# awkrail/svpc

Measured on AMD Instinct MI355X. Metric: train steps/sec (vivt, batch=16, clip_seq=12), higher is better.
Workload: dtype bf16x3; 1 GPU; MODEL_TYPE=vivt train step: N=16 videos/GPU x S=12 clips x Lv=100 frames x F=3072, Lt=22, D=768, H=12, L=6 (enc+step-enc+dec), V=951, A=384, E=10; dropout .1/.1/.4; fwd+bwd+allreduce+clip+BertAdam; mode=bf16x3, global_batch=16, parallelism=dp1, launch=hipGraph replay, gpus_requested=1

## Files before the change

include/svpc_hip.h:

```cpp
#ifndef SVPC_HIP_H
#define SVPC_HIP_H
#include <stddef.h>
#ifdef __cplusplus
extern "C" {
#endif

typedef struct ihipStream_t* svpc_stream_t;
typedef unsigned long long svpc_u64;

#define SVPC_ACT_NONE 0
#define SVPC_ACT_RELU 1
#define SVPC_ACT_GELU 2
#define SVPC_ACT_SIGMOID 3

const char* svpc_last_error(void);
int svpc_abi_version(void);

int svpc_ln_fwd(const float* x, const int* src_rows, const float* res, const float* gamma, const float* beta, float* y,
                float* mean, float* rstd, int R, int D, float eps, float p_pre, unsigned site_pre, float p_post,
                unsigned site_post, const svpc_u64* seed, const float* add1, int mod1, const float* add2, const int* idx2,
                svpc_stream_t stream);
int svpc_ln_fwd_t(const void* x, int x_dt, const int* src_rows, const void* res, const float* gamma, const float* beta, void* y,
                  int y_dt, float* mean, float* rstd, int R, int D, float eps, float p_pre, unsigned site_pre, float p_post,
                  unsigned site_post, const svpc_u64* seed, const float* add1, int mod1, const float* add2, const int* idx2,
// ... 46 lines not shown
                   int K, const float* bias, int act, float p_drop, unsigned site, const svpc_u64* seed, int accumulate,
                   float* workspace, size_t workspace_bytes, svpc_stream_t stream);
int svpc_gemm_glds_r(const void* A, int lda, int a_kc, const void* B, int ldb, int b_kc, void* C, int c_dt, int ldc, void* Z, const void* R,
                     int M, int N, int K, const float* bias, int act, float p_drop, unsigned site, const svpc_u64* seed, int accumulate,
                     float* workspace, size_t workspace_bytes, svpc_stream_t stream);
int svpc_gemm_glds_rg(const void* A, int lda, int a_kc, const void* B, int ldb, int b_kc, void* C, int c_dt, int ldc, void* Z, const void* R,
                      const void* G, int gact, int M, int N, int K, const float* bias, int act, float p_drop, unsigned site,
                      const svpc_u64* seed, int accumulate, float* workspace, size_t workspace_bytes, svpc_stream_t stream);
int svpc_gemm_p8(const void* A, int lda, const void* B, int ldb, void* C, int ldc, void* Z, int M, int N, int K, const float* bias, int act,
                 svpc_stream_t stream);
int svpc_gemm_p8x3_supported(int lda, int a_lo, int ldb, int ldc, int c_lo, int ldz, int M, int N, int K);
int svpc_gemm_p8x3(const void* A, int lda, int a_lo, const void* B, int ldb, long long b_lo, void* C, int ldc, int c_lo, void* Z, int ldz,
                   int M, int N, int K, const float* bias, int act, svpc_stream_t stream);
int svpc_gemm_s4x3(const void* A, int lda, int a_lo, const void* B, int ldb, long long b_lo, void* C, int ldc, int c_lo, void* Z, int ldz,
                   int M, int N, int K, const float* bias, int act, svpc_stream_t stream);
int svpc_gemm_s4t_supported(int lda, int ldb, int ldc, int M, int N, int K);
int svpc_gemm_s4t(const void* A, int lda, const void* B, int ldb, void* C, int ldc, const void* R, int M, int N, int K, svpc_stream_t stream);
int svpc_gemm_p8t_supported(int lda, int ldb, int ldc, int M, int N, int K);
int svpc_gemm_p8t(const void* A, int lda, const void* B, int ldb, void* C, int ldc, const void* G, int gact, const void* R, int M, int N, int K,
                  svpc_stream_t stream);
int svpc_gemm_l32_supported(int a_kc, int b_kc, int lda, int ldb, int M, int N, int K);
int svpc_gemm_l32_preferred(int a_kc, int b_kc, int lda, int ldb, int M, int N, int K);
int svpc_gemm_l32(const float* A, int lda, int a_kc, const float* B, int ldb, int b_kc, float* C, int ldc, float* Z, int M, int N, int K,
                  const float* bias, int act, float p_drop, unsigned site, const svpc_u64* seed, int accumulate, float* workspace,
                  size_t workspace_bytes, svpc_stream_t stream);
int svpc_gemm_l32_r(const float* A, int lda, int a_kc, const float* B, int ldb, int b_kc, float* C, int ldc, float* Z, const float* R, int M,
                    int N, int K, const float* bias, int act, float p_drop, unsigned site, const svpc_u64* seed, int accumulate,
                    float* workspace, size_t workspace_bytes, svpc_stream_t stream);
int svpc_gemm_l32_rg(const float* A, int lda, int a_kc, const float* B, int ldb, int b_kc, float* C, int ldc, const float* R, const float* G,
                     int gact, int M, int N, int K, int accumulate, float* workspace, size_t workspace_bytes, svpc_stream_t stream);
int svpc_gemm_l32_x3(const float* A, int lda, int a_kc, const float* B, int ldb, int b_kc, float* C, int ldc, float* Z, const float* R, int M,
                     int N, int K, const float* bias, int act, float p_drop, unsigned site, const svpc_u64* seed, int accumulate,
// ... 300 lines not shown
```

svpc_amd/csrc/gemm_s4t.hip:

```cpp
#include "gemm_common.h"
#include <stdlib.h>

typedef __bf16 bf16x8 __attribute__((ext_vector_type(8)));
typedef float floatx4 __attribute__((ext_vector_type(4)));
typedef short short4s __attribute__((ext_vector_type(4)));
typedef const void __attribute__((address_space(1))) * s4t_gptr;
typedef void __attribute__((address_space(3))) * s4t_lptr;

constexpr int S4T_BK = 64;
constexpr int S4T_HALF = 128 * S4T_BK * 2;
constexpr int S4T_STAGE = 2 * S4T_HALF;

__device__ __forceinline__ bf16x8 s4t_frag_tr(const char* __restrict__ a) {
    typedef short4s __attribute__((address_space(3))) * lds_ptr;
    const short4s lo = __builtin_amdgcn_ds_read_tr16_b64_v4i16((lds_ptr)(a));
    const short4s hi = __builtin_amdgcn_ds_read_tr16_b64_v4i16((lds_ptr)(a + 4 * 256));
    union { short s[8]; bf16x8 v; } u;
    u.s[0] = lo[0]; u.s[1] = lo[1]; u.s[2] = lo[2]; u.s[3] = lo[3];
    u.s[4] = hi[0]; u.s[5] = hi[1]; u.s[6] = hi[2]; u.s[7] = hi[3];
    return u.v;
}

template <bool HASR, int NS>
__global__ __launch_bounds__(512, NS == 2 ? 2 : 1) void gemm_s4t_kernel(const __bf16* __restrict__ A, int lda, const __bf16* __restrict__ B, int ldb,
                                                                        __bf16* __restrict__ C, int ldc, const __bf16* __restrict__ R, int M,
                                                                        int N, int K, int tiles_m, int tiles_n, int remap) {
    __shared__ __attribute__((aligned(1024))) char smem[NS * S4T_STAGE];
    const int wg = remap ? xcd_remap(blockIdx.x, tiles_m * tiles_n) : (int)blockIdx.x;
    const int tm = wg / tiles_n, tn = wg - tm * tiles_n;
    const int m0 = tm * 128, n0 = tn * 128;
    const int nk = K / S4T_BK;
    const int lane = threadIdx.x & 63, wave = __builtin_amdgcn_readfirstlane(threadIdx.x >> 6);
    const int wr = wave >> 1, wc = wave & 1;

    const int sr = lane >> 2, sc = (lane & 3) ^ (((lane >> 5) & 1) << 1);
    const __bf16* const ga = A + (size_t)min(m0 + 16 * wave + sr, M - 1) * lda + 8 * sc;
    const __bf16* gb[2];
#pragma unroll
    for (int u = 0; u < 2; ++u) {
        const int kr = 8 * wave + 4 * u + (lane >> 4);
        const int fx = 2 * ((kr & 3) | ((kr >> 1) & 4));
        const int col = min(n0 + 8 * ((lane & 15) ^ fx), N - 8);
        gb[u] = B + (size_t)kr * ldb + col;
    }
    const size_t stepB = (size_t)S4T_BK * ldb;
#define S4T_ISSUE(t)                                                                                                              \
    do {                                                                                                                          \
        char* st_ = smem + ((t) % NS) * S4T_STAGE;                                                                                \
        const __bf16* sa_ = ga + (size_t)(t) * S4T_BK;                                                                            \
        __builtin_amdgcn_global_load_lds((s4t_gptr)(sa_), (s4t_lptr)(st_ + ((wave * 2) << 10)), 16, 0, 0);                        \
        __builtin_amdgcn_global_load_lds((s4t_gptr)(sa_ + 32), (s4t_lptr)(st_ + ((wave * 2 + 1) << 10)), 16, 0, 0);               \
        __builtin_amdgcn_global_load_lds((s4t_gptr)(gb[0] + (size_t)(t) * stepB), (s4t_lptr)(st_ + S4T_HALF + wave * 2048), 16, 0, 0);        \
        __builtin_amdgcn_global_load_lds((s4t_gptr)(gb[1] + (size_t)(t) * stepB), (s4t_lptr)(st_ + S4T_HALF + wave * 2048 + 1024), 16, 0, 0); \
    } while (0)
    const int fr_off = (lane & 15) * 64 + ((((lane >> 4) ^ (((lane >> 3) & 1) << 1))) << 4);
#define S4T_FRAGA(img, blk, kb) (*reinterpret_cast<const bf16x8*>((img) + (((blk) * 2 + (kb)) << 10) + fr_off))
    const int tg = lane >> 4, tq = (lane & 15) >> 2, tp = lane & 3;
    const int tfx = 2 * (tq + 4 * (tg & 1));
    const int tb_off = (8 * tg + tq) * 256 + ((tp & 1) << 3);
    const int tp1 = tp >> 1;
#define S4T_FRAGB(img, cb, kb) s4t_frag_tr((img) + (kb) * (32 * 256) + tb_off + (((((2 * (cb)) ^ tfx)) | tp1) << 4))

    floatx4 acc[2][4];
#pragma unroll
    for (int i = 0; i < 2; ++i)
#pragma unroll
        for (int j = 0; j < 4; ++j) acc[i][j] = floatx4{0.f, 0.f, 0.f, 0.f};

#pragma unroll
    for (int t = 0; t < NS - 1; ++t)
        if (t < nk) S4T_ISSUE(t);
    for (int t = 0; t < nk; ++t) {
        if (NS == 4 && t + 2 < nk) asm volatile("s_waitcnt vmcnt(8)" ::: "memory");
        else if (NS >= 3 && t + 1 < nk) asm volatile("s_waitcnt vmcnt(4)" ::: "memory");
        else asm volatile("s_waitcnt vmcnt(0)" ::: "memory");
        __builtin_amdgcn_s_barrier();
        __builtin_amdgcn_sched_barrier(0);
        if (t + NS - 1 < nk) S4T_ISSUE(t + NS - 1);
        const char* sa = smem + (t % NS) * S4T_STAGE;
        const char* sb = sa + S4T_HALF;
#pragma unroll
        for (int kb = 0; kb < 2; ++kb) {
            bf16x8 bfr[4], afr[2];
#pragma unroll
            for (int j = 0; j < 4; ++j) bfr[j] = S4T_FRAGB(sb, wc * 4 + j, kb);
#pragma unroll
            for (int i = 0; i < 2; ++i) afr[i] = S4T_FRAGA(sa, wr * 2 + i, kb);
#pragma unroll
            for (int i = 0; i < 2; ++i)
#pragma unroll
                for (int j = 0; j < 4; ++j) acc[i][j] = __builtin_amdgcn_mfma_f32_16x16x32_bf16(bfr[j], afr[i], acc[i][j], 0, 0, 0);
        }
    }
#undef S4T_ISSUE
#undef S4T_FRAGA
#undef S4T_FRAGB
    __syncthreads();
    char* wl = smem + wave * 8192;
    const int row0 = m0 + wr * 32, col0 = n0 + wc * 64;
    const int l15 = lane & 15, q = lane >> 4;
    const int c8 = lane & 7, cc = col0 + 8 * c8, r0 = lane >> 3;
    const bool col_ok = cc + 8 <= N;
    bf16x8 rv[HASR ? 4 : 1];
#pragma unroll
    for (int it = 0; it < 4; ++it) {
        const int r = it * 8 + r0;
        if (HASR && col_ok && row0 + r < M) rv[it] = *reinterpret_cast<const bf16x8*>(R + (size_t)(row0 + r) * ldc + cc);
    }
#pragma unroll
    for (int i = 0; i < 2; ++i) {
        const int r = i * 16 + l15;
#pragma unroll
        for (int j = 0; j < 4; ++j) {
            const int c16 = j * 4 + q;
            *reinterpret_cast<floatx4*>(wl + r * 256 + ((c16 ^ (r & 7)) << 4)) = acc[i][j];
        }
    }
#pragma unroll
    for (int it = 0; it < 4; ++it) {
        const int r = it * 8 + r0;
        const floatx4 v0 = *reinterpret_cast<const floatx4*>(wl + r * 256 + (((2 * c8) ^ (r & 7)) << 4));
        const floatx4 v1 = *reinterpret_cast<const floatx4*>(wl + r * 256 + (((2 * c8 + 1) ^ (r & 7)) << 4));
        float v[8] = {v0[0], v0[1], v0[2], v0[3], v1[0], v1[1], v1[2], v1[3]};
        if (col_ok && row0 + r < M) {
            const size_t o = (size_t)(row0 + r) * ldc + cc;
            if (HASR) {
#pragma unroll
                for (int j = 0; j < 8; ++j) v[j] += (float)rv[it][j];
            }
            bf16x8 ov;
#pragma unroll
            for (int j = 0; j < 8; ++j) ov[j] = (__bf16)v[j];
            *reinterpret_cast<bf16x8*>(C + o) = ov;
        }
    }
}

extern "C" {

int svpc_gemm_s4t_supported(int lda, int ldb, int ldc, int M, int N, int K) {
    if (M <= 0 || N < 8 || K < S4T_BK || K % S4T_BK != 0 || (N & 7) != 0) return 0;
    if ((lda & 7) || (ldb & 7) || (ldc & 7) || lda < K || ldb < N || ldc < N) return 0;
    return 1;
}

int svpc_gemm_s4t(const void* A, int lda, const void* B, int ldb, void* C, int ldc, const void* R, int M, int N, int K, hipStream_t stream) {
    if (M <= 0 || N <= 0) return 0;
    SVPC_REQUIRE(svpc_gemm_s4t_supported(lda, ldb, ldc, M, N, K) == 1 &&
                     ((((uintptr_t)A) | ((uintptr_t)B) | ((uintptr_t)C) | ((uintptr_t)R)) & 15) == 0,
                 "gemm_s4t: needs K % 64 == 0, N % 8 == 0, 16-byte aligned bf16 rows");
    static int remap = -1, deep_max = -1;
    if (remap < 0) { const char* e = getenv("SVPC_GEMM_REMAP"); remap = e ? atoi(e) : 1; }
    if (deep_max < 0) { const char* e = getenv("SVPC_S4T_DEEP_MAX"); deep_max = e ? atoi(e) : 256; }
    const int tiles_m = ceil_div(M, 128), tiles_n = ceil_div(N, 128);
    const bool deep = tiles_m * tiles_n <= deep_max;
#define S4T_GO(RV, NSV)                                                                                                           \
    hipLaunchKernelGGL((gemm_s4t_kernel<RV, NSV>), dim3(tiles_m * tiles_n), dim3(512), 0, stream, (const __bf16*)A, lda, (const __bf16*)B, \
                       ldb, (__bf16*)C, ldc, (const __bf16*)R, M, N, K, tiles_m, tiles_n, remap)
    if (R != nullptr) { if (deep) S4T_GO(true, 4); else S4T_GO(true, 2); }
    else { if (deep) S4T_GO(false, 4); else S4T_GO(false, 2); }
#undef S4T_GO
    return svpc_check_launch("gemm_s4t");
}

}
```

svpc_amd/csrc/gemm_s4x3.hip:

```cpp
#include "gemm_common.h"
#include <stdlib.h>

typedef __bf16 bf16x8 __attribute__((ext_vector_type(8)));
typedef float floatx4 __attribute__((ext_vector_type(4)));
typedef const void __attribute__((address_space(1))) * s4_gptr;
typedef void __attribute__((address_space(3))) * s4_lptr;

constexpr int S4_BK = 64;
constexpr int S4_KS = 32;
constexpr int S4_HALF = 128 * S4_BK * 2;
constexpr int S4_STAGE = 2 * S4_HALF;

__device__ __forceinline__ uint32_t s4_pack2(float lo, float hi) {
    union { __bf16 h[2]; uint32_t u; } pk;
    pk.h[0] = (__bf16)lo; pk.h[1] = (__bf16)hi;
    return pk.u;
}
__device__ __forceinline__ float s4_lo(float v) { return v - (float)(__bf16)v; }
__device__ __forceinline__ float s4_gelu(float x) {
    const float u = x * 0.70710678118654752f, au = fabsf(u);
    const float t = __builtin_amdgcn_rcpf(fmaf(0.3275911f, au, 1.0f));
    float p = fmaf(1.061405429f, t, -1.453152027f);
    p = fmaf(p, t, 1.421413741f);
    p = fmaf(p, t, -0.284496736f);
    p = fmaf(p, t, 0.254829592f);
    const float e = __expf(-au * au);
    return 0.5f * x * (1.0f + copysignf(fmaf(-p * t, e, 1.0f), u));
}
template <int ACT>
__device__ __forceinline__ float s4_act(float z) {
    if (ACT == ACT_RELU) return fmaxf(z, 0.f);
    if (ACT == ACT_GELU) return s4_gelu(z);
    return z;
}

template <int ACT, int MODE>
__device__ __forceinline__ void s4_store_pass(const floatx4 (&acc)[2][4], __bf16* __restrict__ C, int ldc, const float4 (&bb)[4], int row0,
                                              int col0, int M, int N, int lane, char* __restrict__ wl) {
    const int l15 = lane & 15, q = lane >> 4;
#pragma unroll
    for (int i = 0; i < 2; ++i) {
        const int r = i * 16 + l15;
#pragma unroll
        for (int j = 0; j < 4; ++j) {
            float z0 = acc[i][j][0] + bb[j].x, z1 = acc[i][j][1] + bb[j].y, z2 = acc[i][j][2] + bb[j].z, z3 = acc[i][j][3] + bb[j].w;
            if (MODE != 0) { z0 = s4_act<ACT>(z0); z1 = s4_act<ACT>(z1); z2 = s4_act<ACT>(z2); z3 = s4_act<ACT>(z3); }
            if (MODE == 2) { z0 = s4_lo(z0); z1 = s4_lo(z1); z2 = s4_lo(z2); z3 = s4_lo(z3); }
            uint2 v;
            v.x = s4_pack2(z0, z1); v.y = s4_pack2(z2, z3);
            const int c16 = j * 2 + (q >> 1);
            *reinterpret_cast<uint2*>(wl + r * 128 + ((c16 ^ (r & 7)) << 4) + ((q & 1) << 3)) = v;
        }
    }
    const int chunk = lane & 7, cc = col0 + 8 * chunk, r0 = lane >> 3;
    uint32_t off = ((uint32_t)(row0 + r0) * (uint32_t)ldc + (uint32_t)cc) * 2u;
    const uint32_t step = 16u * (uint32_t)ldc;
    const bool col_ok = cc + 8 <= N;
#pragma unroll
    for (int it = 0; it < 4; ++it) {
        const int r = it * 8 + r0;
        const uint4 v = *reinterpret_cast<const uint4*>(wl + r * 128 + ((chunk ^ (r & 7)) << 4));
        if (col_ok && row0 + r < M) *reinterpret_cast<uint4*>(reinterpret_cast<char*>(C) + off) = v;
        off += step;
    }
}

template <int ACT, bool HASZ, int NS>
__global__ __launch_bounds__(512, NS == 2 ? 2 : 1) void gemm_s4x3_kernel(const __bf16* __restrict__ A, int lda, int a_lo, const __bf16* __restrict__ B, int ldb,
                                                           long long b_lo, __bf16* __restrict__ C, int ldc, int c_lo, __bf16* __restrict__ Z,
                                                           int ldz, const float* __restrict__ bias, int M, int N, int K, int tiles_m,
                                                           int tiles_n, int remap) {
    __shared__ __attribute__((aligned(1024))) char smem[NS * S4_STAGE];
    const int wg = remap ? xcd_remap(blockIdx.x, tiles_m * tiles_n) : (int)blockIdx.x;
    const int tm = wg / tiles_n, tn = wg - tm * tiles_n;
    const int m0 = tm * 128, n0 = tn * 128;
    const int nk = K / S4_KS;
    const int lane = threadIdx.x & 63, wave = __builtin_amdgcn_readfirstlane(threadIdx.x >> 6);
    const int wr = wave >> 1, wc = wave & 1;

    const int sr = lane >> 2, sc = (lane & 3) ^ (((lane >> 5) & 1) << 1);
    const __bf16* const ga = A + (size_t)min(m0 + 16 * wave + sr, M - 1) * lda + 8 * sc;
    const __bf16* const gb = B + (size_t)min(n0 + 16 * wave + sr, N - 1) * ldb + 8 * sc;
#define S4_ISSUE(t)                                                                                                               \
    do {                                                                                                                          \
        char* da_ = smem + ((t) % NS) * S4_STAGE + ((wave * 2) << 10);                                                            \
        const size_t o_ = (size_t)(t) * S4_KS;                                                                                    \
        __builtin_amdgcn_global_load_lds((s4_gptr)(ga + o_), (s4_lptr)(da_), 16, 0, 0);                                           \
        __builtin_amdgcn_global_load_lds((s4_gptr)(ga + o_ + a_lo), (s4_lptr)(da_ + 1024), 16, 0, 0);                             \
        __builtin_amdgcn_global_load_lds((s4_gptr)(gb + o_), (s4_lptr)(da_ + S4_HALF), 16, 0, 0);                                 \
        __builtin_amdgcn_global_load_lds((s4_gptr)(gb + o_ + b_lo), (s4_lptr)(da_ + S4_HALF + 1024), 16, 0, 0);                   \
    } while (0)
    const int fr_off = (lane & 15) * 64 + ((((lane >> 4) ^ (((lane >> 3) & 1) << 1))) << 4);
#define S4_FRAG(img, blk, kb) (*reinterpret_cast<const bf16x8*>((img) + (((blk) * 2 + (kb)) << 10) + fr_off))

    floatx4 acc[2][4];
#pragma unroll
    for (int i = 0; i < 2; ++i)
#pragma unroll
        for (int j = 0; j < 4; ++j) acc[i][j] = floatx4{0.f, 0.f, 0.f, 0.f};

#pragma unroll
    for (int t = 0; t < NS - 1; ++t)
        if (t < nk) S4_ISSUE(t);
    for (int t = 0; t < nk; ++t) {
        if (NS == 4 && t + 2 < nk) asm volatile("s_waitcnt vmcnt(8)" ::: "memory");
        else if (NS >= 3 && t + 1 < nk) asm volatile("s_waitcnt vmcnt(4)" ::: "memory");
        else asm volatile("s_waitcnt vmcnt(0)" ::: "memory");
        __builtin_amdgcn_s_barrier();
        __builtin_amdgcn_sched_barrier(0);
        if (t + NS - 1 < nk) S4_ISSUE(t + NS - 1);
        const char* sa = smem + (t % NS) * S4_STAGE;
        const char* sb = sa + S4_HALF;
        bf16x8 bfr[2][4], afr[2][2];
#pragma unroll
        for (int pl = 0; pl < 2; ++pl) {
#pragma unroll
            for (int j = 0; j < 4; ++j) bfr[pl][j] = S4_FRAG(sb, wc * 4 + j, pl);
#pragma unroll
            for (int i = 0; i < 2; ++i) afr[pl][i] = S4_FRAG(sa, wr * 2 + i, pl);
        }
#pragma unroll
        for (int term = 0; term < 3; ++term)
#pragma unroll
            for (int i = 0; i < 2; ++i)
#pragma unroll
                for (int j = 0; j < 4; ++j)
                    acc[i][j] = __builtin_amdgcn_mfma_f32_16x16x32_bf16(bfr[term == 2 ? 1 : 0][j], afr[term == 0 ? 1 : 0][i], acc[i][j], 0, 0, 0);
    }
#undef S4_ISSUE
#undef S4_FRAG
    __syncthreads();
    char* wl = smem + wave * 4096;
    const int row0 = m0 + wr * 32, col0 = n0 + wc * 64;
    float4 bb[4];
#pragma unroll
    for (int j = 0; j < 4; ++j) {
        const int c = col0 + j * 16 + 4 * (lane >> 4);
        bb[j] = (bias && c + 4 <= N) ? *reinterpret_cast<const float4*>(bias + c) : make_float4(0.f, 0.f, 0.f, 0.f);
    }
    if (HASZ) s4_store_pass<ACT, 0>(acc, Z, ldz, bb, row0, col0, M, N, lane, wl);
    s4_store_pass<ACT, 2>(acc, C + c_lo, ldc, bb, row0, col0, M, N, lane, wl);
    s4_store_pass<ACT, 1>(acc, C, ldc, bb, row0, col0, M, N, lane, wl);
}

extern "C" {

int svpc_gemm_s4x3(const void* A, int lda, int a_lo, const void* B, int ldb, long long b_lo, void* C, int ldc, int c_lo, void* Z, int ldz,
                   int M, int N, int K, const float* bias, int act, hipStream_t stream) {
    if (M <= 0 || N <= 0) return 0;
    if (Z == nullptr) ldz = 0;
    SVPC_REQUIRE(K >= 2 * S4_KS && K % S4_KS == 0 && (N & 7) == 0 && !((lda | a_lo | ldb | ldc | c_lo | ldz) & 7) && a_lo >= K && lda >= a_lo + K &&
                     c_lo >= N && ldc >= c_lo + N && ldb >= K && (b_lo & 7) == 0 &&
                     (unsigned long long)M * (unsigned long long)ldc * 2ull < (1ull << 32) &&
                     ((((uintptr_t)A) | ((uintptr_t)B) | ((uintptr_t)C) | ((uintptr_t)Z) | ((uintptr_t)bias)) & 15) == 0 &&
                     (act == ACT_RELU || act == ACT_GELU || (act == ACT_NONE && Z == nullptr)) && (Z == nullptr || ldz >= N),
                 "gemm_s4x3: needs K % 32 == 0, K >= 64, N % 8 == 0, 16-byte aligned split rows (lo plane behind the hi plane), act in {none, relu, gelu}");
    static int remap = -1;
    if (remap < 0) { const char* e = getenv("SVPC_GEMM_REMAP"); remap = e ? atoi(e) : 1; }
    const int tiles_m = ceil_div(M, 128), tiles_n = ceil_div(N, 128);
    static int deep_max = -1;
    if (deep_max < 0) { const char* e = getenv("SVPC_S4X3_DEEP_MAX"); deep_max = e ? atoi(e) : 256; }
    const bool deep = tiles_m * tiles_n <= deep_max;
#define S4_GO(ACTV, ZV)                                                                                                           \
    do {                                                                                                                          \
        if (deep) hipLaunchKernelGGL((gemm_s4x3_kernel<ACTV, ZV, 4>), dim3(tiles_m * tiles_n), dim3(512), 0, stream, (const __bf16*)A, lda, a_lo, \
                       (const __bf16*)B, ldb, b_lo, (__bf16*)C, ldc, c_lo, (__bf16*)Z, ldz, bias, M, N, K, tiles_m, tiles_n, remap); \
        else hipLaunchKernelGGL((gemm_s4x3_kernel<ACTV, ZV, 2>), dim3(tiles_m * tiles_n), dim3(512), 0, stream, (const __bf16*)A, lda, a_lo, \
                       (const __bf16*)B, ldb, b_lo, (__bf16*)C, ldc, c_lo, (__bf16*)Z, ldz, bias, M, N, K, tiles_m, tiles_n, remap); \
    } while (0)
    const bool z = Z != nullptr;
    if (act == ACT_GELU) { if (z) S4_GO(ACT_GELU, true); else S4_GO(ACT_GELU, false); }
    else if (act == ACT_RELU) { if (z) S4_GO(ACT_RELU, true); else S4_GO(ACT_RELU, false); }
    else S4_GO(ACT_NONE, false);
#undef S4_GO
    return svpc_check_launch("gemm_s4x3");
}

}
```

Baseline: 90.40 steps/s (one step = 16 clip-sequences per GPU; whole-job aggregate).

## Add 96-row/column tile variants to s4x3 and s4t GEMMs with CU-aware picker

Templates the split-bf16x3 and transposed s4t GEMM kernels on tile shape (128 or 96 in each dimension), with wave count, per-wave fragment counts, DMA unit assignment and epilogue indexing derived from the shape. A picker chooses the smallest tile that still fits the tile count within the device CU count, so small text GEMMs launch more workgroups and fill more CUs. The cost is smaller tiles with less reuse per workgroup, extra DMA bookkeeping, and a variable vmcnt wait through a switch.

```diff
diff --git a/include/svpc_hip.h b/include/svpc_hip.h
--- a/include/svpc_hip.h
+++ b/include/svpc_hip.h
@@ -84,8 +84,13 @@
                    int M, int N, int K, const float* bias, int act, svpc_stream_t stream);
 int svpc_gemm_s4x3(const void* A, int lda, int a_lo, const void* B, int ldb, long long b_lo, void* C, int ldc, int c_lo, void* Z, int ldz,
                    int M, int N, int K, const float* bias, int act, svpc_stream_t stream);
+int svpc_text_gemm_tile(int kernel, int M, int N, int cus);
+int svpc_gemm_s4x3_tile(const void* A, int lda, int a_lo, const void* B, int ldb, long long b_lo, void* C, int ldc, int c_lo, void* Z, int ldz,
+                        int M, int N, int K, const float* bias, int act, int bm, int bn, svpc_stream_t stream);
 int svpc_gemm_s4t_supported(int lda, int ldb, int ldc, int M, int N, int K);
 int svpc_gemm_s4t(const void* A, int lda, const void* B, int ldb, void* C, int ldc, const void* R, int M, int N, int K, svpc_stream_t stream);
+int svpc_gemm_s4t_tile(const void* A, int lda, const void* B, int ldb, void* C, int ldc, const void* R, int M, int N, int K, int bm, int bn,
+                       svpc_stream_t stream);
 int svpc_gemm_p8t_supported(int lda, int ldb, int ldc, int M, int N, int K);
 int svpc_gemm_p8t(const void* A, int lda, const void* B, int ldb, void* C, int ldc, const void* G, int gact, const void* R, int M, int N, int K,
                   svpc_stream_t stream);
diff --git a/svpc_amd/csrc/gemm_s4t.hip b/svpc_amd/csrc/gemm_s4t.hip
--- a/svpc_amd/csrc/gemm_s4t.hip
+++ b/svpc_amd/csrc/gemm_s4t.hip
@@ -1,4 +1,5 @@
 #include "gemm_common.h"
+#include "text_gemm_tiles.h"
 #include <stdlib.h>
 
 typedef __bf16 bf16x8 __attribute__((ext_vector_type(8)));
@@ -9,7 +10,6 @@
 
 constexpr int S4T_BK = 64;
 constexpr int S4T_HALF = 128 * S4T_BK * 2;
-constexpr int S4T_STAGE = 2 * S4T_HALF;
 
 __device__ __forceinline__ bf16x8 s4t_frag_tr(const char* __restrict__ a) {
     typedef short4s __attribute__((address_space(3))) * lds_ptr;
@@ -21,37 +21,80 @@
     return u.v;
 }
 
-template <bool HASR, int NS>
-__global__ __launch_bounds__(512, NS == 2 ? 2 : 1) void gemm_s4t_kernel(const __bf16* __restrict__ A, int lda, const __bf16* __restrict__ B, int ldb,
-                                                                        __bf16* __restrict__ C, int ldc, const __bf16* __restrict__ R, int M,
-                                                                        int N, int K, int tiles_m, int tiles_n, int remap) {
-    __shared__ __attribute__((aligned(1024))) char smem[NS * S4T_STAGE];
+template <int BM, int BN> struct S4TShape {
+    static_assert((BM == 128 || BM == 96) && (BN == 128 || BN == 96), "gemm_s4t: tile shapes are 128 / 96 rows by 128 / 96 columns");
+    static constexpr int NW = (BM == 96 && BN == 96) ? 4 : 8;
+    static constexpr int TI = BM == 96 ? 3 : 2;
+    static constexpr int WN = (BM == 96 && BN == 128) ? 4 : 2;
+    static constexpr int TJ = BN / 16 / WN;
+    static constexpr int NU = BM / 16 + 8;
+    static constexpr int UPW = (NU + NW - 1) / NW;
+    static constexpr int STAGE = BM * S4T_BK * 2 + S4T_HALF;
+    static_assert((BM / 16) % TI == 0 && (BM / 16 / TI) * WN == NW, "wave map");
+};
+
+__device__ __forceinline__ void s4t_wait_vm(int n) {
+    switch (n) {
+        case 0: asm volatile("s_waitcnt vmcnt(0)" ::: "memory"); break;
+        case 2: asm volatile("s_waitcnt vmcnt(2)" ::: "memory"); break;
+        case 4: asm volatile("s_waitcnt vmcnt(4)" ::: "memory"); break;
+        case 6: asm volatile("s_waitcnt vmcnt(6)" ::: "memory"); break;
+        case 8: asm volatile("s_waitcnt vmcnt(8)" ::: "memory"); break;
+        case 12: asm volatile("s_waitcnt vmcnt(12)" ::: "memory"); break;
+        case 16: asm volatile("s_waitcnt vmcnt(16)" ::: "memory"); break;
+        default: asm volatile("s_waitcnt vmcnt(0)" ::: "memory"); break;
+    }
+}
+
+template <bool HASR, int NS, int BM, int BN>
+__global__ __launch_bounds__((S4TShape<BM, BN>::NW * 64), NS == 2 ? 2 : 1) void gemm_s4t_kernel(
+    const __bf16* __restrict__ A, int lda, const __bf16* __restrict__ B, int ldb, __bf16* __restrict__ C, int ldc, const __bf16* __restrict__ R,
+    int M, int N, int K, int tiles_m, int tiles_n, int remap) {
+    using SH = S4TShape<BM, BN>;
+    constexpr int NW = SH::NW, TI = SH::TI, TJ = SH::TJ, WN = SH::WN, NU = SH::NU, UPW = SH::UPW, STAGE = SH::STAGE, RBA = BM / 16;
+    constexpr int HALF_A = BM * S4T_BK * 2;
+    static_assert(NS * STAGE >= NW * TI * 16 * 256, "the epilogue images reuse the stages");
+    __shared__ __attribute__((aligned(1024))) char smem[NS * STAGE];
     const int wg = remap ? xcd_remap(blockIdx.x, tiles_m * tiles_n) : (int)blockIdx.x;
     const int tm = wg / tiles_n, tn = wg - tm * tiles_n;
-    const int m0 = tm * 128, n0 = tn * 128;
+    const int m0 = tm * BM, n0 = tn * BN;
     const int nk = K / S4T_BK;
     const int lane = threadIdx.x & 63, wave = __builtin_amdgcn_readfirstlane(threadIdx.x >> 6);
-    const int wr = wave >> 1, wc = wave & 1;
+    const int wr = wave / WN, wc = wave - wr * WN;
 
     const int sr = lane >> 2, sc = (lane & 3) ^ (((lane >> 5) & 1) << 1);
-    const __bf16* const ga = A + (size_t)min(m0 + 16 * wave + sr, M - 1) * lda + 8 * sc;
-    const __bf16* gb[2];
-#pragma unroll
-    for (int u = 0; u < 2; ++u) {
-        const int kr = 8 * wave + 4 * u + (lane >> 4);
-        const int fx = 2 * ((kr & 3) | ((kr >> 1) & 4));
-        const int col = min(n0 + 8 * ((lane & 15) ^ fx), N - 8);
-        gb[u] = B + (size_t)kr * ldb + col;
-    }
-    const size_t stepB = (size_t)S4T_BK * ldb;
+    const __bf16* gsrc[UPW][2];
+    size_t gstep[UPW];
+    bool gon[UPW][2];
+    int n_dma = 0;
+#pragma unroll
+    for (int u = 0; u < UPW; ++u) {
+        const int unit = wave + NW * u;
+        const bool is_a = NW * (u + 1) <= RBA ? true : (NW * u >= RBA ? false : unit < RBA);
+        const bool valid = NW * (u + 1) <= NU ? true : unit < NU;
+        const __bf16* const pa = A + (size_t)min(m0 + 16 * unit + sr, M - 1) * lda + 8 * sc;
+#pragma unroll
+        for (int h = 0; h < 2; ++h) {
+            const int kr = 8 * max(unit - RBA, 0) + 4 * h + (lane >> 4);
+            const int ch = (lane & 15) ^ (2 * ((kr & 3) | ((kr >> 1) & 4)));
+            const int col = min(n0 + 8 * ch, N - 8);
+            gsrc[u][h] = is_a ? pa + 32 * h : B + (size_t)kr * ldb + col;
+            gon[u][h] = BN == 128 || is_a || ch < BN / 8;
+        }
+        gstep[u] = is_a ? (size_t)S4T_BK : (size_t)S4T_BK * ldb;
+        if (valid) n_dma += 2;
+    }
 #define S4T_ISSUE(t)                                                                                                              \
     do {                                                                                                                          \
-        char* st_ = smem + ((t) % NS) * S4T_STAGE;                                                                                \
-        const __bf16* sa_ = ga + (size_t)(t) * S4T_BK;                                                                            \
-        __builtin_amdgcn_global_load_lds((s4t_gptr)(sa_), (s4t_lptr)(st_ + ((wave * 2) << 10)), 16, 0, 0);                        \
-        __builtin_amdgcn_global_load_lds((s4t_gptr)(sa_ + 32), (s4t_lptr)(st_ + ((wave * 2 + 1) << 10)), 16, 0, 0);               \
-        __builtin_amdgcn_global_load_lds((s4t_gptr)(gb[0] + (size_t)(t) * stepB), (s4t_lptr)(st_ + S4T_HALF + wave * 2048), 16, 0, 0);        \
-        __builtin_amdgcn_global_load_lds((s4t_gptr)(gb[1] + (size_t)(t) * stepB), (s4t_lptr)(st_ + S4T_HALF + wave * 2048 + 1024), 16, 0, 0); \
+        _Pragma("unroll") for (int u_ = 0; u_ < UPW; ++u_) {                                                                      \
+            const int unit_ = wave + NW * u_;                                                                                     \
+            if (NW * (u_ + 1) <= NU || unit_ < NU) {                                                                              \
+                char* da_ = smem + ((t) % NS) * STAGE + unit_ * 2048;                                                             \
+                const size_t o_ = (size_t)(t) * gstep[u_];                                                                        \
+                if (BN == 128 || gon[u_][0]) __builtin_amdgcn_global_load_lds((s4t_gptr)(gsrc[u_][0] + o_), (s4t_lptr)(da_), 16, 0, 0);          \
+                if (BN == 128 || gon[u_][1]) __builtin_amdgcn_global_load_lds((s4t_gptr)(gsrc[u_][1] + o_), (s4t_lptr)(da_ + 1024), 16, 0, 0);   \
+            }                                                                                                                     \
+        }                                                                                                                         \
     } while (0)
     const int fr_off = (lane & 15) * 64 + ((((lane >> 4) ^ (((lane >> 3) & 1) << 1))) << 4);
 #define S4T_FRAGA(img, blk, kb) (*reinterpret_cast<const bf16x8*>((img) + (((blk) * 2 + (kb)) << 10) + fr_off))
@@ -61,69 +104,72 @@
     const int tp1 = tp >> 1;
 #define S4T_FRAGB(img, cb, kb) s4t_frag_tr((img) + (kb) * (32 * 256) + tb_off + (((((2 * (cb)) ^ tfx)) | tp1) << 4))
 
-    floatx4 acc[2][4];
-#pragma unroll
-    for (int i = 0; i < 2; ++i)
-#pragma unroll
-        for (int j = 0; j < 4; ++j) acc[i][j] = floatx4{0.f, 0.f, 0.f, 0.f};
+    floatx4 acc[TI][TJ];
+#pragma unroll
+    for (int i = 0; i < TI; ++i)
+#pragma unroll
+        for (int j = 0; j < TJ; ++j) acc[i][j] = floatx4{0.f, 0.f, 0.f, 0.f};
 
 #pragma unroll
     for (int t = 0; t < NS - 1; ++t)
         if (t < nk) S4T_ISSUE(t);
     for (int t = 0; t < nk; ++t) {
-        if (NS == 4 && t + 2 < nk) asm volatile("s_waitcnt vmcnt(8)" ::: "memory");
-        else if (NS >= 3 && t + 1 < nk) asm volatile("s_waitcnt vmcnt(4)" ::: "memory");
-        else asm volatile("s_waitcnt vmcnt(0)" ::: "memory");
+        if (NS == 4 && t + 2 < nk) s4t_wait_vm(2 * n_dma);
+        else if (NS >= 3 && t + 1 < nk) s4t_wait_vm(n_dma);
+        else s4t_wait_vm(0);
         __builtin_amdgcn_s_barrier();
         __builtin_amdgcn_sched_barrier(0);
         if (t + NS - 1 < nk) S4T_ISSUE(t + NS - 1);
-        const char* sa = smem + (t % NS) * S4T_STAGE;
-        const char* sb = sa + S4T_HALF;
+        const char* sa = smem + (t % NS) * STAGE;
+        const char* sb = sa + HALF_A;
 #pragma unroll
         for (int kb = 0; kb < 2; ++kb) {
-            bf16x8 bfr[4], afr[2];
-#pragma unroll
-            for (int j = 0; j < 4; ++j) bfr[j] = S4T_FRAGB(sb, wc * 4 + j, kb);
-#pragma unroll
-            for (int i = 0; i < 2; ++i) afr[i] = S4T_FRAGA(sa, wr * 2 + i, kb);
-#pragma unroll
-            for (int i = 0; i < 2; ++i)
-#pragma unroll
-                for (int j = 0; j < 4; ++j) acc[i][j] = __builtin_amdgcn_mfma_f32_16x16x32_bf16(bfr[j], afr[i], acc[i][j], 0, 0, 0);
+            bf16x8 bfr[TJ], afr[TI];
+#pragma unroll
+            for (int j = 0; j < TJ; ++j) bfr[j] = S4T_FRAGB(sb, wc * TJ + j, kb);
+#pragma unroll
+            for (int i = 0; i < TI; ++i) afr[i] = S4T_FRAGA(sa, wr * TI + i, kb);
+#pragma unroll
+            for (int i = 0; i < TI; ++i)
+#pragma unroll
+                for (int j = 0; j < TJ; ++j) acc[i][j] = __builtin_amdgcn_mfma_f32_16x16x32_bf16(bfr[j], afr[i], acc[i][j], 0, 0, 0);
         }
     }
 #undef S4T_ISSUE
 #undef S4T_FRAGA
 #undef S4T_FRAGB
     __syncthreads();
-    char* wl = smem + wave * 8192;
-    const int row0 = m0 + wr * 32, col0 = n0 + wc * 64;
+    char* wl = smem + wave * (TI * 16 * 256);
+    const int row0 = m0 + wr * (16 * TI), col0 = n0 + wc * (16 * TJ);
     const int l15 = lane & 15, q = lane >> 4;
-    const int c8 = lane & 7, cc = col0 + 8 * c8, r0 = lane >> 3;
-    const bool col_ok = cc + 8 <= N;
-    bf16x8 rv[HASR ? 4 : 1];
-#pragma unroll
-    for (int it = 0; it < 4; ++it) {
-        const int r = it * 8 + r0;
-        if (HASR && col_ok && row0 + r < M) rv[it] = *reinterpret_cast<const bf16x8*>(R + (size_t)(row0 + r) * ldc + cc);
-    }
-#pragma unroll
-    for (int i = 0; i < 2; ++i) {
+    constexpr int CG = 2 * TJ, NCH = TI * 16 * CG, ITERS = (NCH + 63) / 64;
+    int er[ITERS], ec[ITERS];
+    bool eok[ITERS];
+    bf16x8 rv[HASR ? ITERS : 1];
+#pragma unroll
+    for (int it = 0; it < ITERS; ++it) {
+        const int idx = NCH % 64 == 0 ? it * 64 + lane : min(it * 64 + lane, NCH - 1);
+        er[it] = idx / CG; ec[it] = idx - er[it] * CG;
+        eok[it] = (NCH % 64 == 0 || it * 64 + lane < NCH) && col0 + 8 * ec[it] + 8 <= N && row0 + er[it] < M;
+        if (HASR) rv[it] = *reinterpret_cast<const bf16x8*>(R + (size_t)min(row0 + er[it], M - 1) * ldc + min(col0 + 8 * ec[it], N - 8));
+    }
+#pragma unroll
+    for (int i = 0; i < TI; ++i) {
         const int r = i * 16 + l15;
 #pragma unroll
-        for (int j = 0; j < 4; ++j) {
+        for (int j = 0; j < TJ; ++j) {
             const int c16 = j * 4 + q;
             *reinterpret_cast<floatx4*>(wl + r * 256 + ((c16 ^ (r & 7)) << 4)) = acc[i][j];
         }
     }
 #pragma unroll
-    for (int it = 0; it < 4; ++it) {
-        const int r = it * 8 + r0;
+    for (int it = 0; it < ITERS; ++it) {
+        const int r = er[it], c8 = ec[it];
         const floatx4 v0 = *reinterpret_cast<const floatx4*>(wl + r * 256 + (((2 * c8) ^ (r & 7)) << 4));
         const floatx4 v1 = *reinterpret_cast<const floatx4*>(wl + r * 256 + (((2 * c8 + 1) ^ (r & 7)) << 4));
         float v[8] = {v0[0], v0[1], v0[2], v0[3], v1[0], v1[1], v1[2], v1[3]};
-        if (col_ok && row0 + r < M) {
-            const size_t o = (size_t)(row0 + r) * ldc + cc;
+        if (eok[it]) {
+            const size_t o = (size_t)(row0 + r) * ldc + col0 + 8 * c8;
             if (HASR) {
 #pragma unroll
                 for (int j = 0; j < 8; ++j) v[j] += (float)rv[it][j];
@@ -134,6 +180,14 @@
             *reinterpret_cast<bf16x8*>(C + o) = ov;
         }
     }
+}
+
+template <bool HASR, int NS, int BM, int BN>
+static void s4t_launch(const void* A, int lda, const void* B, int ldb, void* C, int ldc, const void* R, int M, int N, int K, int remap,
+                       hipStream_t stream) {
+    const int tiles_m = ceil_div(M, BM), tiles_n = ceil_div(N, BN);
+    hipLaunchKernelGGL((gemm_s4t_kernel<HASR, NS, BM, BN>), dim3(tiles_m * tiles_n), dim3(S4TShape<BM, BN>::NW * 64), 0, stream, (const __bf16*)A,
+                       lda, (const __bf16*)B, ldb, (__bf16*)C, ldc, (const __bf16*)R, M, N, K, tiles_m, tiles_n, remap);
 }
 
 extern "C" {
@@ -144,23 +198,37 @@
     return 1;
 }
 
-int svpc_gemm_s4t(const void* A, int lda, const void* B, int ldb, void* C, int ldc, const void* R, int M, int N, int K, hipStream_t stream) {
+int svpc_gemm_s4t_tile(const void* A, int lda, const void* B, int ldb, void* C, int ldc, const void* R, int M, int N, int K, int bm, int bn,
+                       hipStream_t stream) {
     if (M <= 0 || N <= 0) return 0;
     SVPC_REQUIRE(svpc_gemm_s4t_supported(lda, ldb, ldc, M, N, K) == 1 &&
                      ((((uintptr_t)A) | ((uintptr_t)B) | ((uintptr_t)C) | ((uintptr_t)R)) & 15) == 0,
                  "gemm_s4t: needs K % 64 == 0, N % 8 == 0, 16-byte aligned bf16 rows");
+    if (bm == 0 && bn == 0) {
+        const int i = svpc_text_tile_pick(SVPC_TEXT_GEMM_S4T, M, N, svpc_text_tile_cus());
+        bm = SVPC_TEXT_TILE_BM[i]; bn = SVPC_TEXT_TILE_BN[i];
+    }
+    SVPC_REQUIRE((bm == 128 || bm == 96) && (bn == 128 || bn == 96), "gemm_s4t: tile shapes are 128 / 96 rows by 128 / 96 columns");
     static int remap = -1, deep_max = -1;
     if (remap < 0) { const char* e = getenv("SVPC_GEMM_REMAP"); remap = e ? atoi(e) : 1; }
     if (deep_max < 0) { const char* e = getenv("SVPC_S4T_DEEP_MAX"); deep_max = e ? atoi(e) : 256; }
-    const int tiles_m = ceil_div(M, 128), tiles_n = ceil_div(N, 128);
-    const bool deep = tiles_m * tiles_n <= deep_max;
-#define S4T_GO(RV, NSV)                                                                                                           \
-    hipLaunchKernelGGL((gemm_s4t_kernel<RV, NSV>), dim3(tiles_m * tiles_n), dim3(512), 0, stream, (const __bf16*)A, lda, (const __bf16*)B, \
-                       ldb, (__bf16*)C, ldc, (const __bf16*)R, M, N, K, tiles_m, tiles_n, remap)
-    if (R != nullptr) { if (deep) S4T_GO(true, 4); else S4T_GO(true, 2); }
-    else { if (deep) S4T_GO(false, 4); else S4T_GO(false, 2); }
+    const bool deep = ceil_div(M, 128) * ceil_div(N, 128) <= deep_max;
+#define S4T_ARGS A, lda, B, ldb, C, ldc, R, M, N, K, remap, stream
+#define S4T_GO(RV)                                                                                                                \
+    do {                                                                                                                          \
+        if (bm == 128 && bn == 128) { if (deep) s4t_launch<RV, 4, 128, 128>(S4T_ARGS); else s4t_launch<RV, 2, 128, 128>(S4T_ARGS); } \
+        else if (bm == 96 && bn == 128) s4t_launch<RV, 4, 96, 128>(S4T_ARGS);                                                     \
+        else if (bm == 128 && bn == 96) s4t_launch<RV, 4, 128, 96>(S4T_ARGS);                                                     \
+        else s4t_launch<RV, 4, 96, 96>(S4T_ARGS);                                                                                 \
+    } while (0)
+    if (R != nullptr) S4T_GO(true); else S4T_GO(false);
 #undef S4T_GO
+#undef S4T_ARGS
     return svpc_check_launch("gemm_s4t");
 }
 
-}
+int svpc_gemm_s4t(const void* A, int lda, const void* B, int ldb, void* C, int ldc, const void* R, int M, int N, int K, hipStream_t stream) {
+    return svpc_gemm_s4t_tile(A, lda, B, ldb, C, ldc, R, M, N, K, 0, 0, stream);
+}
+
+}
diff --git a/svpc_amd/csrc/gemm_s4x3.hip b/svpc_amd/csrc/gemm_s4x3.hip
--- a/svpc_amd/csrc/gemm_s4x3.hip
+++ b/svpc_amd/csrc/gemm_s4x3.hip
@@ -1,4 +1,5 @@
 #include "gemm_common.h"
+#include "text_gemm_tiles.h"
 #include <stdlib.h>
 
 typedef __bf16 bf16x8 __attribute__((ext_vector_type(8)));
@@ -8,8 +9,6 @@
 
 constexpr int S4_BK = 64;
 constexpr int S4_KS = 32;
-constexpr int S4_HALF = 128 * S4_BK * 2;
-constexpr int S4_STAGE = 2 * S4_HALF;
 
 __device__ __forceinline__ uint32_t s4_pack2(float lo, float hi) {
     union { __bf16 h[2]; uint32_t u; } pk;
@@ -34,15 +33,39 @@
     return z;
 }
 
-template <int ACT, int MODE>
-__device__ __forceinline__ void s4_store_pass(const floatx4 (&acc)[2][4], __bf16* __restrict__ C, int ldc, const float4 (&bb)[4], int row0,
+template <int BM, int BN> struct S4Shape {
+    static_assert((BM == 128 || BM == 96) && (BN == 128 || BN == 96), "gemm_s4x3: tile shapes are 128 / 96 rows by 128 / 96 columns");
+    static constexpr int NW = (BM == 96 && BN == 96) ? 4 : 8;
+    static constexpr int TI = BM == 96 ? 3 : 2;
+    static constexpr int WN = (BM == 96 && BN == 128) ? 4 : 2;
+    static constexpr int TJ = BN / 16 / WN;
+    static constexpr int NU = BM / 16 + BN / 16;
+    static constexpr int UPW = (NU + NW - 1) / NW;
+    static constexpr int STAGE = (BM + BN) * S4_BK * 2;
+    static_assert((BM / 16) % TI == 0 && (BM / 16 / TI) * WN == NW, "wave map");
+};
+
+__device__ __forceinline__ void s4_wait_vm(int n) {
+    switch (n) {
+        case 0: asm volatile("s_waitcnt vmcnt(0)" ::: "memory"); break;
+        case 2: asm volatile("s_waitcnt vmcnt(2)" ::: "memory"); break;
+        case 4: asm volatile("s_waitcnt vmcnt(4)" ::: "memory"); break;
+        case 6: asm volatile("s_waitcnt vmcnt(6)" ::: "memory"); break;
+        case 8: asm volatile("s_waitcnt vmcnt(8)" ::: "memory"); break;
+        case 12: asm volatile("s_waitcnt vmcnt(12)" ::: "memory"); break;
+        default: asm volatile("s_waitcnt vmcnt(0)" ::: "memory"); break;
+    }
+}
+
+template <int ACT, int MODE, int TI, int TJ>
+__device__ __forceinline__ void s4_store_pass(const floatx4 (&acc)[TI][TJ], __bf16* __restrict__ C, int ldc, const float4 (&bb)[TJ], int row0,
                                               int col0, int M, int N, int lane, char* __restrict__ wl) {
     const int l15 = lane & 15, q = lane >> 4;
 #pragma unroll
-    for (int i = 0; i < 2; ++i) {
+    for (int i = 0; i < TI; ++i) {
         const int r = i * 16 + l15;
 #pragma unroll
-        for (int j = 0; j < 4; ++j) {
+        for (int j = 0; j < TJ; ++j) {
             float z0 = acc[i][j][0] + bb[j].x, z1 = acc[i][j][1] + bb[j].y, z2 = acc[i][j][2] + bb[j].z, z3 = acc[i][j][3] + bb[j].w;
             if (MODE != 0) { z0 = s4_act<ACT>(z0); z1 = s4_act<ACT>(z1); z2 = s4_act<ACT>(z2); z3 = s4_act<ACT>(z3); }
             if (MODE == 2) { z0 = s4_lo(z0); z1 = s4_lo(z1); z2 = s4_lo(z2); z3 = s4_lo(z3); }
@@ -52,101 +75,131 @@
             *reinterpret_cast<uint2*>(wl + r * 128 + ((c16 ^ (r & 7)) << 4) + ((q & 1) << 3)) = v;
         }
     }
-    const int chunk = lane & 7, cc = col0 + 8 * chunk, r0 = lane >> 3;
-    uint32_t off = ((uint32_t)(row0 + r0) * (uint32_t)ldc + (uint32_t)cc) * 2u;
-    const uint32_t step = 16u * (uint32_t)ldc;
-    const bool col_ok = cc + 8 <= N;
-#pragma unroll
-    for (int it = 0; it < 4; ++it) {
-        const int r = it * 8 + r0;
+    constexpr int CPR = 2 * TJ, NCH = TI * 16 * CPR;
+#pragma unroll
+    for (int it = 0; it < (NCH + 63) / 64; ++it) {
+        const int idx = NCH % 64 == 0 ? it * 64 + lane : min(it * 64 + lane, NCH - 1), r = idx / CPR, chunk = idx - r * CPR, cc = col0 + 8 * chunk;
         const uint4 v = *reinterpret_cast<const uint4*>(wl + r * 128 + ((chunk ^ (r & 7)) << 4));
-        if (col_ok && row0 + r < M) *reinterpret_cast<uint4*>(reinterpret_cast<char*>(C) + off) = v;
-        off += step;
-    }
-}
-
-template <int ACT, bool HASZ, int NS>
-__global__ __launch_bounds__(512, NS == 2 ? 2 : 1) void gemm_s4x3_kernel(const __bf16* __restrict__ A, int lda, int a_lo, const __bf16* __restrict__ B, int ldb,
-                                                           long long b_lo, __bf16* __restrict__ C, int ldc, int c_lo, __bf16* __restrict__ Z,
-                                                           int ldz, const float* __restrict__ bias, int M, int N, int K, int tiles_m,
-                                                           int tiles_n, int remap) {
-    __shared__ __attribute__((aligned(1024))) char smem[NS * S4_STAGE];
+        const uint32_t off = ((uint32_t)(row0 + r) * (uint32_t)ldc + (uint32_t)cc) * 2u;
+        if ((NCH % 64 == 0 || it * 64 + lane < NCH) && cc + 8 <= N && row0 + r < M) *reinterpret_cast<uint4*>(reinterpret_cast<char*>(C) + off) = v;
+    }
+}
+
+template <int ACT, bool HASZ, int NS, int BM, int BN>
+__global__ __launch_bounds__((S4Shape<BM, BN>::NW * 64), NS == 2 ? 2 : 1) void gemm_s4x3_kernel(
+    const __bf16* __restrict__ A, int lda, int a_lo, const __bf16* __restrict__ B, int ldb, long long b_lo, __bf16* __restrict__ C, int ldc,
+    int c_lo, __bf16* __restrict__ Z, int ldz, const float* __restrict__ bias, int M, int N, int K, int tiles_m, int tiles_n, int remap) {
+    using SH = S4Shape<BM, BN>;
+    constexpr int NW = SH::NW, TI = SH::TI, TJ = SH::TJ, WN = SH::WN, NU = SH::NU, UPW = SH::UPW, STAGE = SH::STAGE, RBA = BM / 16;
+    constexpr int HALF_A = BM * S4_BK * 2;
+    static_assert(NS * STAGE >= NW * TI * 16 * 128, "the epilogue images reuse the stages");
+    __shared__ __attribute__((aligned(1024))) char smem[NS * STAGE];
     const int wg = remap ? xcd_remap(blockIdx.x, tiles_m * tiles_n) : (int)blockIdx.x;
     const int tm = wg / tiles_n, tn = wg - tm * tiles_n;
-    const int m0 = tm * 128, n0 = tn * 128;
+    const int m0 = tm * BM, n0 = tn * BN;
     const int nk = K / S4_KS;
     const int lane = threadIdx.x & 63, wave = __builtin_amdgcn_readfirstlane(threadIdx.x >> 6);
-    const int wr = wave >> 1, wc = wave & 1;
+    const int wr = wave / WN, wc = wave - wr * WN;
 
     const int sr = lane >> 2, sc = (lane & 3) ^ (((lane >> 5) & 1) << 1);
-    const __bf16* const ga = A + (size_t)min(m0 + 16 * wave + sr, M - 1) * lda + 8 * sc;
-    const __bf16* const gb = B + (size_t)min(n0 + 16 * wave + sr, N - 1) * ldb + 8 * sc;
+    const __bf16* gsrc[UPW];
+    long long glo[UPW];
+    int n_dma = 0;
+#pragma unroll
+    for (int u = 0; u < UPW; ++u) {
+        const int unit = wave + NW * u;
+        const bool is_a = NW * (u + 1) <= RBA ? true : (NW * u >= RBA ? false : unit < RBA);
+        const bool valid = NW * (u + 1) <= NU ? true : unit < NU;
+        const __bf16* const pa = A + (size_t)min(m0 + 16 * unit + sr, M - 1) * lda + 8 * sc;
+        const __bf16* const pb = B + (size_t)min(n0 + 16 * max(unit - RBA, 0) + sr, N - 1) * ldb + 8 * sc;
+        gsrc[u] = is_a ? pa : pb;
+        glo[u] = is_a ? (long long)a_lo : b_lo;
+        if (valid) n_dma += 2;
+    }
 #define S4_ISSUE(t)                                                                                                               \
     do {                                                                                                                          \
-        char* da_ = smem + ((t) % NS) * S4_STAGE + ((wave * 2) << 10);                                                            \
         const size_t o_ = (size_t)(t) * S4_KS;                                                                                    \
-        __builtin_amdgcn_global_load_lds((s4_gptr)(ga + o_), (s4_lptr)(da_), 16, 0, 0);                                           \
-        __builtin_amdgcn_global_load_lds((s4_gptr)(ga + o_ + a_lo), (s4_lptr)(da_ + 1024), 16, 0, 0);                             \
-        __builtin_amdgcn_global_load_lds((s4_gptr)(gb + o_), (s4_lptr)(da_ + S4_HALF), 16, 0, 0);                                 \
-        __builtin_amdgcn_global_load_lds((s4_gptr)(gb + o_ + b_lo), (s4_lptr)(da_ + S4_HALF + 1024), 16, 0, 0);                   \
+        _Pragma("unroll") for (int u_ = 0; u_ < UPW; ++u_) {                                                                      \
+            const int unit_ = wave + NW * u_;                                                                                     \
+            if (NW * (u_ + 1) <= NU || unit_ < NU) {                                                                              \
+                char* da_ = smem + ((t) % NS) * STAGE + ((unit_ * 2) << 10);                                                      \
+                __builtin_amdgcn_global_load_lds((s4_gptr)(gsrc[u_] + o_), (s4_lptr)(da_), 16, 0, 0);                             \
+                __builtin_amdgcn_global_load_lds((s4_gptr)(gsrc[u_] + o_ + glo[u_]), (s4_lptr)(da_ + 1024), 16, 0, 0);            \
+            }                                                                                                                     \
+        }                                                                                                                         \
     } while (0)
     const int fr_off = (lane & 15) * 64 + ((((lane >> 4) ^ (((lane >> 3) & 1) << 1))) << 4);
 #define S4_FRAG(img, blk, kb) (*reinterpret_cast<const bf16x8*>((img) + (((blk) * 2 + (kb)) << 10) + fr_off))
 
-    floatx4 acc[2][4];
-#pragma unroll
-    for (int i = 0; i < 2; ++i)
-#pragma unroll
-        for (int j = 0; j < 4; ++j) acc[i][j] = floatx4{0.f, 0.f, 0.f, 0.f};
+    floatx4 acc[TI][TJ];
+#pragma unroll
+    for (int i = 0; i < TI; ++i)
+#pragma unroll
+        for (int j = 0; j < TJ; ++j) acc[i][j] = floatx4{0.f, 0.f, 0.f, 0.f};
 
 #pragma unroll
     for (int t = 0; t < NS - 1; ++t)
         if (t < nk) S4_ISSUE(t);
     for (int t = 0; t < nk; ++t) {
-        if (NS == 4 && t + 2 < nk) asm volatile("s_waitcnt vmcnt(8)" ::: "memory");
-        else if (NS >= 3 && t + 1 < nk) asm volatile("s_waitcnt vmcnt(4)" ::: "memory");
-        else asm volatile("s_waitcnt vmcnt(0)" ::: "memory");
+        if (NS == 4 && t + 2 < nk) s4_wait_vm(2 * n_dma);
+        else if (NS >= 3 && t + 1 < nk) s4_wait_vm(n_dma);
+        else s4_wait_vm(0);
         __builtin_amdgcn_s_barrier();
         __builtin_amdgcn_sched_barrier(0);
         if (t + NS - 1 < nk) S4_ISSUE(t + NS - 1);
-        const char* sa = smem + (t % NS) * S4_STAGE;
-        const char* sb = sa + S4_HALF;
-        bf16x8 bfr[2][4], afr[2][2];
+        const char* sa = smem + (t % NS) * STAGE;
+        const char* sb = sa + HALF_A;
+        bf16x8 bfr[2][TJ], afr[2][TI];
 #pragma unroll
         for (int pl = 0; pl < 2; ++pl) {
 #pragma unroll
-            for (int j = 0; j < 4; ++j) bfr[pl][j] = S4_FRAG(sb, wc * 4 + j, pl);
-#pragma unroll
-            for (int i = 0; i < 2; ++i) afr[pl][i] = S4_FRAG(sa, wr * 2 + i, pl);
+            for (int j = 0; j < TJ; ++j) bfr[pl][j] = S4_FRAG(sb, wc * TJ + j, pl);
+#pragma unroll
+            for (int i = 0; i < TI; ++i) afr[pl][i] = S4_FRAG(sa, wr * TI + i, pl);
         }
 #pragma unroll
         for (int term = 0; term < 3; ++term)
 #pragma unroll
-            for (int i = 0; i < 2; ++i)
-#pragma unroll
-                for (int j = 0; j < 4; ++j)
+            for (int i = 0; i < TI; ++i)
+#pragma unroll
+                for (int j = 0; j < TJ; ++j)
                     acc[i][j] = __builtin_amdgcn_mfma_f32_16x16x32_bf16(bfr[term == 2 ? 1 : 0][j], afr[term == 0 ? 1 : 0][i], acc[i][j], 0, 0, 0);
     }
 #undef S4_ISSUE
 #undef S4_FRAG
     __syncthreads();
-    char* wl = smem + wave * 4096;
-    const int row0 = m0 + wr * 32, col0 = n0 + wc * 64;
-    float4 bb[4];
-#pragma unroll
-    for (int j = 0; j < 4; ++j) {
+    char* wl = smem + wave * (TI * 16 * 128);
+    const int row0 = m0 + wr * (16 * TI), col0 = n0 + wc * (16 * TJ);
+    float4 bb[TJ];
+#pragma unroll
+    for (int j = 0; j < TJ; ++j) {
         const int c = col0 + j * 16 + 4 * (lane >> 4);
         bb[j] = (bias && c + 4 <= N) ? *reinterpret_cast<const float4*>(bias + c) : make_float4(0.f, 0.f, 0.f, 0.f);
     }
-    if (HASZ) s4_store_pass<ACT, 0>(acc, Z, ldz, bb, row0, col0, M, N, lane, wl);
-    s4_store_pass<ACT, 2>(acc, C + c_lo, ldc, bb, row0, col0, M, N, lane, wl);
-    s4_store_pass<ACT, 1>(acc, C, ldc, bb, row0, col0, M, N, lane, wl);
+    if (HASZ) s4_store_pass<ACT, 0, TI, TJ>(acc, Z, ldz, bb, row0, col0, M, N, lane, wl);
+    s4_store_pass<ACT, 2, TI, TJ>(acc, C + c_lo, ldc, bb, row0, col0, M, N, lane, wl);
+    s4_store_pass<ACT, 1, TI, TJ>(acc, C, ldc, bb, row0, col0, M, N, lane, wl);
+}
+
+template <int ACT, bool HASZ, int NS, int BM, int BN>
+static void s4x3_launch(const void* A, int lda, int a_lo, const void* B, int ldb, long long b_lo, void* C, int ldc, int c_lo, void* Z, int ldz,
+                        int M, int N, int K, const float* bias, int remap, hipStream_t stream) {
+    const int tiles_m = ceil_div(M, BM), tiles_n = ceil_div(N, BN);
+    hipLaunchKernelGGL((gemm_s4x3_kernel<ACT, HASZ, NS, BM, BN>), dim3(tiles_m * tiles_n), dim3(S4Shape<BM, BN>::NW * 64), 0, stream,
+                       (const __bf16*)A, lda, a_lo, (const __bf16*)B, ldb, b_lo, (__bf16*)C, ldc, c_lo, (__bf16*)Z, ldz, bias, M, N, K, tiles_m,
+                       tiles_n, remap);
 }
 
 extern "C" {
 
-int svpc_gemm_s4x3(const void* A, int lda, int a_lo, const void* B, int ldb, long long b_lo, void* C, int ldc, int c_lo, void* Z, int ldz,
-                   int M, int N, int K, const float* bias, int act, hipStream_t stream) {
+int svpc_text_gemm_tile(int kernel, int M, int N, int cus) {
+    if (kernel != SVPC_TEXT_GEMM_S4X3 && kernel != SVPC_TEXT_GEMM_S4T) return 0;
+    const int i = svpc_text_tile_pick(kernel, M, N, cus);
+    return svpc_text_tile_code(SVPC_TEXT_TILE_BM[i], SVPC_TEXT_TILE_BN[i]);
+}
+
+int svpc_gemm_s4x3_tile(const void* A, int lda, int a_lo, const void* B, int ldb, long long b_lo, void* C, int ldc, int c_lo, void* Z, int ldz,
+                        int M, int N, int K, const float* bias, int act, int bm, int bn, hipStream_t stream) {
     if (M <= 0 || N <= 0) return 0;
     if (Z == nullptr) ldz = 0;
     SVPC_REQUIRE(K >= 2 * S4_KS && K % S4_KS == 0 && (N & 7) == 0 && !((lda | a_lo | ldb | ldc | c_lo | ldz) & 7) && a_lo >= K && lda >= a_lo + K &&
@@ -155,25 +208,36 @@
                      ((((uintptr_t)A) | ((uintptr_t)B) | ((uintptr_t)C) | ((uintptr_t)Z) | ((uintptr_t)bias)) & 15) == 0 &&
                      (act == ACT_RELU || act == ACT_GELU || (act == ACT_NONE && Z == nullptr)) && (Z == nullptr || ldz >= N),
                  "gemm_s4x3: needs K % 32 == 0, K >= 64, N % 8 == 0, 16-byte aligned split rows (lo plane behind the hi plane), act in {none, relu, gelu}");
+    if (bm == 0 && bn == 0) {
+        const int i = svpc_text_tile_pick(SVPC_TEXT_GEMM_S4X3, M, N, svpc_text_tile_cus());
+        bm = SVPC_TEXT_TILE_BM[i]; bn = SVPC_TEXT_TILE_BN[i];
+    }
+    SVPC_REQUIRE((bm == 128 || bm == 96) && (bn == 128 || bn == 96), "gemm_s4x3: tile shapes are 128 / 96 rows by 128 / 96 columns");
     static int remap = -1;
     if (remap < 0) { const char* e = getenv("SVPC_GEMM_REMAP"); remap = e ? atoi(e) : 1; }
-    const int tiles_m = ceil_div(M, 128), tiles_n = ceil_div(N, 128);
     static int deep_max = -1;
     if (deep_max < 0) { const char* e = getenv("SVPC_S4X3_DEEP_MAX"); deep_max = e ? atoi(e) : 256; }
-    const bool deep = tiles_m * tiles_n <= deep_max;
+    const bool deep = ceil_div(M, 128) * ceil_div(N, 128) <= deep_max;
+#define S4_ARGS A, lda, a_lo, B, ldb, b_lo, C, ldc, c_lo, Z, ldz, M, N, K, bias, remap, stream
 #define S4_GO(ACTV, ZV)                                                                                                           \
     do {                                                                                                                          \
-        if (deep) hipLaunchKernelGGL((gemm_s4x3_kernel<ACTV, ZV, 4>), dim3(tiles_m * tiles_n), dim3(512), 0, stream, (const __bf16*)A, lda, a_lo, \
-                       (const __bf16*)B, ldb, b_lo, (__bf16*)C, ldc, c_lo, (__bf16*)Z, ldz, bias, M, N, K, tiles_m, tiles_n, remap); \
-        else hipLaunchKernelGGL((gemm_s4x3_kernel<ACTV, ZV, 2>), dim3(tiles_m * tiles_n), dim3(512), 0, stream, (const __bf16*)A, lda, a_lo, \
-                       (const __bf16*)B, ldb, b_lo, (__bf16*)C, ldc, c_lo, (__bf16*)Z, ldz, bias, M, N, K, tiles_m, tiles_n, remap); \
+        if (bm == 128 && bn == 128) { if (deep) s4x3_launch<ACTV, ZV, 4, 128, 128>(S4_ARGS); else s4x3_launch<ACTV, ZV, 2, 128, 128>(S4_ARGS); } \
+        else if (bm == 96 && bn == 128) s4x3_launch<ACTV, ZV, 4, 96, 128>(S4_ARGS);                                               \
+        else if (bm == 128 && bn == 96) s4x3_launch<ACTV, ZV, 4, 128, 96>(S4_ARGS);                                               \
+        else s4x3_launch<ACTV, ZV, 4, 96, 96>(S4_ARGS);                                                                           \
     } while (0)
     const bool z = Z != nullptr;
     if (act == ACT_GELU) { if (z) S4_GO(ACT_GELU, true); else S4_GO(ACT_GELU, false); }
     else if (act == ACT_RELU) { if (z) S4_GO(ACT_RELU, true); else S4_GO(ACT_RELU, false); }
     else S4_GO(ACT_NONE, false);
 #undef S4_GO
+#undef S4_ARGS
     return svpc_check_launch("gemm_s4x3");
 }
 
-}
+int svpc_gemm_s4x3(const void* A, int lda, int a_lo, const void* B, int ldb, long long b_lo, void* C, int ldc, int c_lo, void* Z, int ldz,
+                   int M, int N, int K, const float* bias, int act, hipStream_t stream) {
+    return svpc_gemm_s4x3_tile(A, lda, a_lo, B, ldb, b_lo, C, ldc, c_lo, Z, ldz, M, N, K, bias, act, 0, 0, stream);
+}
+
+}
diff --git a/svpc_amd/csrc/text_gemm_tiles.h b/svpc_amd/csrc/text_gemm_tiles.h
--- /dev/null
+++ b/svpc_amd/csrc/text_gemm_tiles.h
@@ -0,0 +1,35 @@
+#pragma once
+
+enum { SVPC_TEXT_GEMM_S4X3 = 0, SVPC_TEXT_GEMM_S4T = 1 };
+
+constexpr int SVPC_TEXT_TILES = 4;
+constexpr int SVPC_TEXT_TILE_BM[SVPC_TEXT_TILES] = {128, 96, 128, 96};
+constexpr int SVPC_TEXT_TILE_BN[SVPC_TEXT_TILES] = {128, 128, 96, 96};
+constexpr unsigned SVPC_TEXT_TILE_KEPT[2] = {0xFu, 0x7u};
+
+static inline int svpc_text_tile_code(int bm, int bn) { return (bm << 8) | bn; }
+
+static inline int svpc_text_tile_pick(int kernel, int M, int N, int cus) {
+    int best = 0, best_sum = 0, best_area = 0;
+    bool found = false;
+    for (int i = 0; i < SVPC_TEXT_TILES; ++i) {
+        if (!((SVPC_TEXT_TILE_KEPT[kernel] >> i) & 1u)) continue;
+        const int bm = SVPC_TEXT_TILE_BM[i], bn = SVPC_TEXT_TILE_BN[i];
+        const long long tiles = (long long)((M + bm - 1) / bm) * ((N + bn - 1) / bn);
+        if (tiles > cus) continue;
+        const int sum = bm + bn, area = bm * bn;
+        if (!found || sum < best_sum || (sum == best_sum && area > best_area)) {
+            best = i; best_sum = sum; best_area = area; found = true;
+        }
+    }
+    return best;
+}
+
+static inline int svpc_text_tile_cus() {
+    static int cus = -1;
+    if (cus < 0) {
+        hipDeviceProp_t prop; int dev = 0;
+        cus = (hipGetDevice(&dev) == hipSuccess && hipGetDeviceProperties(&prop, dev) == hipSuccess) ? prop.multiProcessorCount : 256;
+    }
+    return cus;
+}
```

New measurement: 90.80 steps/s (one step = 16 clip-sequences per GPU; whole-job aggregate) (median of 6 runs). Within noise of the previous version (+0.4%).
